# NVIDIA/tacotron2

Hardware: NVIDIA H100
Metric: mel frames/sec (B=64,T_text=150) (higher is better)
Workload: dtype f32 (split-fp16 tensor-core operands hi+lo, fp32 accumulate and state)

## Files before the change

tacotron2_b200/_engine.py:

```python
import contextlib
import ctypes as C
import threading

import torch

from . import _capi


def weight_table_spec(hp):
    E, K = hp.encoder_embedding_dim, hp.encoder_kernel_size
    s = [("embedding.weight", (hp.n_symbols, hp.symbols_embedding_dim))]

    def bn(p, c):
        return [(p + "weight", (c,)), (p + "bias", (c,)), (p + "running_mean", (c,)),
                (p + "running_var", (c,)), (p + "num_batches_tracked", ())]
    for i in range(hp.encoder_n_convolutions):
        p = "encoder.convolutions.%d." % i
        s += [(p + "0.conv.weight", (E, E, K)), (p + "0.conv.bias", (E,))] + bn(p + "1.", E)
    H = E // 2
    for suf in ("", "_reverse"):
        s += [("encoder.lstm.weight_ih_l0" + suf, (4 * H, E)), ("encoder.lstm.weight_hh_l0" + suf, (4 * H, H)),
              ("encoder.lstm.bias_ih_l0" + suf, (4 * H,)), ("encoder.lstm.bias_hh_l0" + suf, (4 * H,))]
    d = "decoder."
    nm = hp.n_mel_channels * hp.n_frames_per_step
# ... 278 lines not shown
        a.seed = next_seed() if seed is None else seed
        if stash is not None:
            a.stash, a.stash_bytes = stash.data_ptr(), stash.numel()
        a.gate_threshold = float(gate_threshold)
        a.score_mask_value = float(score_mask_value)
        a.mel, a.gate, a.align = mel.data_ptr(), gate.data_ptr(), align.data_ptr()
        a.mel_lengths, a.n_steps = mel_lengths.data_ptr(), n_steps.data_ptr()
        a.ws, a.ws_bytes = ws.data_ptr(), ws.numel()
        with torch.cuda.device(self.device):
            _capi.check(L.t2_decoder_run(self.handle, C.byref(a), self._stream()))
        self._last_decoder_args = (a, memory, len32, teacher_prenet, pk, ak, dk, ws, mel, gate, align, mel_lengths, n_steps)
        return mel, gate, align, mel_lengths, n_steps

    def decoder_stream(self, memory, n_steps_cap, prenet_keep=None, gate_threshold=0.5, score_mask_value=-float("inf"),
                       impl=None, seed=None):
        return DecoderStream(self, memory, n_steps_cap, prenet_keep, gate_threshold, score_mask_value,
                             self.impl if impl is None else impl, next_seed() if seed is None else seed)

    def decoder_profile(self):
        a = self._last_decoder_args[0]
        out = (C.c_int64 * 72)()
        _capi.check(_capi.lib().t2_decoder_profile(C.byref(a), out))
        names = ["E0 x2->att gemm", "E0 epilogue(ah)", "B1", "E1 ah->dec/att/q gemm", "B2", "attention", "B3",
                 "E2 ctx gemm", "E2 epilogue(dh)", "B4", "E3 dh gemm", "E3 epilogue(mel/x1)", "B5", "E4 x1 gemm+epi", "B6",
                 "att:im2col", "att:mma", "att:energies", "att:softmax", "att:context"]
        return {names[i]: [int(out[s * 24 + i]) for s in range(3)] for i in range(len(names))}

    def grad_table(self, named_grads):
        ptrs = (C.c_void_p * _capi.T2_NUM_WEIGHTS)()
        for i, (n, _) in enumerate(self.spec):
            t = named_grads.get(n)
            ptrs[i] = t.data_ptr() if t is not None else None
        return ptrs

    def decoder_stash(self, B, T_enc, T_mel):
        return self.stash_buffer("decoder", B, T_enc, T_mel)

    def decoder_backward(self, memory, memory_lengths, teacher_prenet, align, stash, seed, training, att_keep, dec_keep,
                         score_mask_value, d_mel, d_gate, d_align, named_grads):
        L = _capi.lib()
        B, Te = int(memory.shape[0]), int(memory.shape[1])
        T = int(align.shape[1])
        f32 = dict(device=self.device, dtype=torch.float32)
        d_memory = torch.empty(B, Te, self.hp.encoder_embedding_dim, **f32)
        d_prenet = torch.empty(T, B, self.hp.prenet_dim, **f32)
        ws = self._workspace("dec_bwd", L.t2_decoder_backward_workspace_bytes(self.handle, B, Te, T))
        a = _capi.T2DecoderBwdArgs()
        memory = memory.contiguous()
# ... 143 lines not shown
```

tacotron2_b200/csrc/decoder_persistent.cu:

```cuda
#include <stdlib.h>
#include <string.h>

#include <vector>

#include "decoder.h"
#include "gemm_f32.cuh"
#include "umma.cuh"

namespace t2 {

namespace {

constexpr int kG = 128;
constexpr int kThreads = 512;
constexpr int kStages = 4;
constexpr int kMaxStages = 4;
constexpr int kRows = 64;
constexpr int kXChunkBytes = 2 * kRows * kChunkK * 2;
constexpr int kColA = 0, kColD = 32, kColS = 64;
constexpr int kHiCols = 80;
constexpr int kAccPitch = 84;
constexpr int kAccBytes = kRows * kAccPitch * 4;
constexpr int kMmaWgs = 3;
constexpr int kAttRound = 64;
constexpr int kAttPlane = kAttRound * 128;
constexpr int kPaPitch = kAttRound + 4;
constexpr int kPaBytes = kAtt * kPaPitch * 4;
constexpr int kWStageMax = 2 * kHiCols * kChunkK * 2;
constexpr int kStageBytes = kXChunkBytes + kWStageMax;
constexpr int kNumEvents = 5;
constexpr int kPCols = 344;
constexpr int kQCta0 = 0, kQCtas = 16, kX2Cta0 = 16, kX2Ctas = 32, kPCta0 = 48, kPCtas = 43;
constexpr int kWeffBytes = kAtt * kChunkK * 2 * 2;
constexpr unsigned long long kWatchdogCycles = 1ull << 32;

struct EventPlan {
  uint32_t w_off;
  uint32_t w_bytes;
  int32_t nrows;
  int32_t col0;
  int32_t ncons;
  int32_t n[3];
  int32_t chunks;
};
struct CtaPlan {
  EventPlan ev[kNumEvents];
};

struct BwdCta {
  EventPlan ep;
  int32_t chunk0, nchunks;
  int32_t col0, split;
};

struct PersistentPack {
  uint8_t* wimg = nullptr; size_t wimg_bytes = 0;
  CtaPlan* plans = nullptr;
  float* wp_all = nullptr;
  float* bias_p = nullptr;
  float* bias_a = nullptr;
  float* bias_d = nullptr;
  int32_t* rows = nullptr;
  float* weff = nullptr;
  uint8_t* weff_img = nullptr;
  uint8_t* bwd_wimg[2] = {nullptr, nullptr};
  struct BwdCta* bwd_plans[2] = {nullptr, nullptr};
};

__global__ void fuse_prenet_proj_kernel(const float* __restrict__ w1, const float* __restrict__ wp,
                                        const float* __restrict__ bp, float* __restrict__ out_w,
                                        float* __restrict__ out_b) {
  const int r = blockIdx.x;
  for (int c = threadIdx.x; c < kDRnn + kEnc; c += blockDim.x) {
    float s = 0.f;
    for (int k = 0; k < kMel; ++k) s = fmaf(w1[r * kMel + k], wp[(long)k * (kDRnn + kEnc) + c], s);
    out_w[(long)r * (kDRnn + kEnc) + c] = s;
  }
  if (threadIdx.x == 0) {
    float s = 0.f;
    for (int k = 0; k < kMel; ++k) s = fmaf(w1[r * kMel + k], bp[k], s);
    out_b[r] = s;
  }
}

__global__ void fuse_location_kernel(const float* __restrict__ wld, const float* __restrict__ wloc,
// ... 78 lines not shown
  while (!ptx::mbar_try_wait(bar, parity)) {
    if (clock64() - t0 > kWatchdogCycles) watchdog_trap(ctrl, code);
  }
}

__device__ __forceinline__ void arrive_release(unsigned int* cnt) {
  asm volatile("fence.acq_rel.gpu;" ::: "memory");
  asm volatile("red.relaxed.gpu.global.add.u32 [%0], 1;" ::"l"(cnt) : "memory");
}
__device__ __forceinline__ void poll_acquire(unsigned int* cnt, unsigned int target, DecoderCtrl* ctrl, int code) {
  const unsigned long long t0 = clock64();
  while (true) {
    unsigned int c;
    asm volatile("ld.relaxed.gpu.global.u32 %0, [%1];" : "=r"(c) : "l"(cnt) : "memory");
    if ((int)(c - target) >= 0) break;
    if (clock64() - t0 > kWatchdogCycles) watchdog_trap(ctrl, code);
  }
  asm volatile("fence.acq_rel.gpu;" ::: "memory");
}

__device__ __forceinline__ void grid_barrier(DecoderCtrl* ctrl, unsigned int& target) {
  ptx::fence_proxy_async();
  __syncthreads();
  target += gridDim.x;
  if (threadIdx.x == 0) {
    arrive_release(&ctrl->bar_count);
    poll_acquire(&ctrl->bar_count, target, ctrl, 100);
  }
  __syncthreads();
  ptx::fence_proxy_async();
}

__device__ __forceinline__ void grid_arrive(DecoderCtrl* ctrl, unsigned int& target) {
  ptx::fence_proxy_async();
  __syncthreads();
  target += gridDim.x;
  if (threadIdx.x == 0) {
    arrive_release(&ctrl->bar_count);
  }
}
__device__ __forceinline__ void grid_wait(DecoderCtrl* ctrl, unsigned int target) {
  if (threadIdx.x == 0) {
    poll_acquire(&ctrl->bar_count, target, ctrl, 101);
  }
  __syncthreads();
  ptx::fence_proxy_async();
}

constexpr unsigned int kStopFlag = 1u << 24;
__device__ __forceinline__ void signal_counter(unsigned int* cnt, unsigned int inc) {
  ptx::fence_proxy_async();
  __syncthreads();
  if (threadIdx.x == 0) {
    asm volatile("fence.acq_rel.gpu;" ::: "memory");
    asm volatile("red.relaxed.gpu.global.add.u32 [%0], %1;" ::"l"(cnt), "r"(inc) : "memory");
  }
}
__device__ __forceinline__ bool wait_counter(unsigned int* cnt, unsigned int target, int* s_flag, DecoderCtrl* ctrl, int code) {
  if (threadIdx.x == 0) {
// ... 30 lines not shown
  uint8_t* stage0;
  __device__ __forceinline__ uint8_t* stage(uint32_t s) const { return stage0 + s * kStageBytes; }
  uint64_t* full;
  uint64_t* empty;
  uint32_t p_stage, p_phase;
  uint32_t c_stage, c_phase;
  uint64_t pol_x, pol_w;
  uint32_t pre;
  uint32_t ns;
};

__device__ __forceinline__ void prefetch_weights(Ring& rg, const EventPlan& nx, const uint8_t* w_img,
                                                 DecoderCtrl* ctrl) {
  uint32_t s = rg.p_stage, ph = rg.p_phase;
  const uint32_t n = min(rg.ns, (uint32_t)nx.chunks);
  for (uint32_t i = 0; i < n; ++i) {
    mbar_wait(&rg.empty[s], ph ^ 1, ctrl, 205);
    ptx::mbar_arrive_expect_tx(&rg.full[s], kXChunkBytes + nx.w_bytes);
    ptx::bulk_g2s_hint(rg.stage(s) + kXChunkBytes, w_img + nx.w_off + (size_t)i * nx.w_bytes, nx.w_bytes,
                       &rg.full[s], rg.pol_w);
    if (++s == rg.ns) { s = 0; ph ^= 1; }
  }
  rg.pre = n;
}

inline bool event_plan_fits(const EventPlan& ep, bool all_widths) {
  if (ep.ncons < 1 || ep.ncons > kMmaWgs) return false;
  for (int c = 0; c < ep.ncons; ++c)
    if (ep.n[c] != 16 && ep.n[c] != 32 && !(all_widths && (ep.n[c] == 8 || ep.n[c] == 24))) return false;
  return true;
}
inline void plan_one_matrix(EventPlan& ep, int rows) {
  ep.ncons = 0; ep.nrows = rows;
  for (int r = rows; r > 0 && ep.ncons < 3; ) {
    const int n = ep.ncons < 2 && r >= 32 ? 32 : r;
    ep.n[ep.ncons++] = n; r -= n;
  }
  ep.w_bytes = (uint32_t)rows * 256;
}
__device__ __forceinline__ void plan_image_rows(const EventPlan& ep, int r, int& hi, int& lo) {
  int roff = 0;
  for (int c = 0; c < ep.ncons; ++c) {
    if (r < ep.n[c]) { hi = roff + r; lo = hi + ep.n[c]; return; }
    r -= ep.n[c]; roff += 2 * ep.n[c];
  }
  hi = lo = 0;
// ... 113 lines not shown
}

__device__ __forceinline__ void acc_take8(float* s_acc, int row, int base, int col, float* s) {
  float* a = s_acc + row * kAccPitch + base + col;
#pragma unroll
  for (int i = 0; i < 8; ++i) { s[i] = a[i]; a[i] = 0.f; }
}

__device__ __forceinline__ void stash_lstm(float* gates, float* cs, float* hs, int t, int Btot, int b, int unit0,
                                           const float (&sg)[4][2], const float (&c)[2], const float (&h)[2]) {
  float* gp = gates + ((long)t * Btot + b) * (4 * kARnn) + unit0;
#pragma unroll
  for (int g = 0; g < 4; ++g) *reinterpret_cast<float2*>(gp + g * kARnn) = make_float2(sg[g][0], sg[g][1]);
  const long o = ((long)(t + 1) * Btot + b) * kARnn + unit0;
  *reinterpret_cast<float2*>(cs + o) = make_float2(c[0], c[1]);
  *reinterpret_cast<float2*>(hs + o) = make_float2(h[0], h[1]);
}

struct KParams {
  const CtaPlan* plans;
  const uint8_t* wimg;
  const float* bias_a; const float* bias_d; const float* bias_p;
  const uint8_t* weff_img; const float* w_v;
  const float* memory; const float* pm; const int32_t* mem_len;
  const uint8_t* prenet_keep; const uint8_t* att_keep; const uint8_t* dec_keep;
  uint8_t* x2_img; uint8_t* ah_img; uint8_t* ctx_img; uint8_t* dh_img; uint8_t* x1_img;
  const uint8_t* teacher_x2_img;
  float* q;
  float* mel; float* gate; float* align; int32_t* mel_lengths; int32_t* n_steps;
  DecoderCtrl* ctrl;
  int B, T, cap, infer, training;
  int nstages;
  int b0, Btot;
  float gate_threshold, score_mask_value, p_att, p_dec;
  uint64_t seed;
  DecoderStash st;
  int t_begin, t_end;
  float* rs_acc;
  float* rs_cell;
  float* rs_att;
  int32_t* rs_done;
  int32_t* rs_status;
};

__device__ __forceinline__ void store_split2(uint8_t* img, int row, int k, float v0, float v1) {
  const int chunk = k >> 6, kc = k & 63;
  __half h0, l0, h1, l1;
  split_fp16(v0, h0, l0);
  split_fp16(v1, h1, l1);
  __half* hi = reinterpret_cast<__half*>(img + (size_t)chunk * kXChunkBytes);
  __half* lo = hi + kRows * kChunkK;
  const uint32_t e = img_elem_offset(row, kc);
  *reinterpret_cast<__half2*>(hi + e) = __halves2half2(h0, h1);
  *reinterpret_cast<__half2*>(lo + e) = __halves2half2(l0, l1);
}

__global__ void __launch_bounds__(kThreads, 1) decoder_persistent_kernel(const KParams p) {
  extern __shared__ __align__(1024) uint8_t smem_raw[];
  const int tid = threadIdx.x, warp = tid >> 5, lane = tid & 31;
  const int cta = blockIdx.x;
  const int T = p.T, TP = T + kLocK - 1;
  const int ntiles = (T + 127) >> 7;

  uint8_t* sp = smem_raw;
  Ring rg;
  rg.ns = (uint32_t)p.nstages;
  rg.stage0 = sp; sp += p.nstages * kStageBytes;
  uint8_t* s_weff = sp; sp += kWeffBytes;
  float* s_acc = reinterpret_cast<float*>(sp); sp += kAccBytes;
  uint64_t* bars = reinterpret_cast<uint64_t*>(sp); sp += 16 * sizeof(uint64_t);
  rg.full = bars; rg.empty = bars + kMaxStages;
  int* s_live = reinterpret_cast<int*>(sp); sp += 16;
  int* s_flag = s_live + 1;
  float* s_bias_a = reinterpret_cast<float*>(sp); sp += 32 * 4;
  float* s_bias_d = reinterpret_cast<float*>(sp); sp += 32 * 4;
  float* s_v = reinterpret_cast<float*>(sp); sp += kAtt * 4;
  float* s_q = reinterpret_cast<float*>(sp); sp += kAtt * 4;
  float* s_red = reinterpret_cast<float*>(sp); sp += 32 * 4;
  uint32_t* s_mask = reinterpret_cast<uint32_t*>(sp); sp += kRows * 4;
  float* s_bias_p = reinterpret_cast<float*>(sp); sp += 8 * 4;
  long long* s_prof = reinterpret_cast<long long*>(sp); sp += 24 * 8;
  float* s_pad0 = reinterpret_cast<float*>(sp); sp += ((TP + 3) & ~3) * 4;
  float* s_pad1 = reinterpret_cast<float*>(sp); sp += ((TP + 3) & ~3) * 4;
// ... 23 lines not shown
    s_pad0[i] = resume ? p.rs_att[((size_t)cta * 2 + 0) * tpp + i] : 0.f;
    s_pad1[i] = resume ? p.rs_att[((size_t)cta * 2 + 1) * tpp + i] : 0.f;
  }
  const CtaPlan& plan = p.plans[cta];
  DecoderCtrl* ctrl = p.ctrl;
  const bool has_p = cta >= kPCta0 && cta < kPCta0 + kPCtas;
  const bool gate_cta = has_p && (cta - kPCta0) * 8 <= kMel && (cta - kPCta0) * 8 + 8 > kMel;
  if (resume && gate_cta && tid < p.B) ctrl->done[tid] = p.rs_done[tid];
  ptx::fence_proxy_async();
  __syncthreads();

  unsigned int bar_target = 0;
  const int quad = warp & 3, cg = warp >> 2;
  const int row = (quad & 1) * 32 + lane;
  const bool is_lo = quad >= 2;
  const bool erow = !is_lo && row < p.B;
  float c_att[2] = {0.f, 0.f}, c_dec[2] = {0.f, 0.f};
  float4* rs_cell = resume ? reinterpret_cast<float4*>(p.rs_cell) + ((size_t)cta * 4 + cg) * kRows + row : nullptr;
  if (resume && !is_lo) {
    const float4 c = *rs_cell;
    c_att[0] = c.x; c_att[1] = c.y; c_dec[0] = c.z; c_dec[1] = c.w;
  }
  const bool has_q = cta >= kQCta0 && cta < kQCta0 + kQCtas;
  const bool has_x2 = cta >= kX2Cta0 && cta < kX2Cta0 + kX2Ctas;
  const int halfk = (kLocK - 1) / 2;
  const int prof_slot = cta == 0 ? 0 : (cta == 60 ? 1 : (cta == 100 ? 2 : -1));
  long long prof_last = clock64();
  if (tid < 24) s_prof[tid] = 0;
#define T2_PROF(ph)                                                        \
  do {                                                                     \
    if (prof_slot >= 0 && tid == 0) {                                      \
      const long long now_ = clock64();                                    \
      s_prof[ph] += now_ - prof_last;    \
      prof_last = now_;                                                    \
    }                                                                      \
  } while (0)
#define T2_TAKE_GATES(colbase, g)                          \
  do {                                                     \
    if (!is_lo) acc_take8(s_acc, row, (colbase), cg * 8, g); \
  } while (0)

  auto x2_epilogue = [&]() {
    float g[8];
    if (cg == 0 && !is_lo) acc_take8(s_acc, row, kColS, 0, g);
    if (cg == 0 && erow) {
      const int col0 = (cta - kX2Cta0) * 8;
      float r[8];
      const uint32_t bits = s_mask[row];
#pragma unroll
      for (int j = 0; j < 8; ++j)
        r[j] = ((bits >> j) & 1u) ? fmaxf(g[j], 0.f) * 2.f : 0.f;
#pragma unroll
      for (int j = 0; j < 8; j += 2) store_split2(p.x2_img, row, col0 + j, r[j], r[j + 1]);
    }
  };

  int t = p.t_begin;
  for (; t < p.t_end; ++t) {
    {
      const uint8_t* x2 = p.infer ? p.x2_img : p.teacher_x2_img + (size_t)t * 4 * kXChunkBytes;
      run_event(rg, plan.ev[0], x2, p.wimg, 4, s_acc, ctrl, &plan.ev[1]);
      T2_PROF(0);
      float g[8];
      T2_TAKE_GATES(kColA, g);
      if (erow) {
        float hv[2], sg[4][2];
#pragma unroll
        for (int u = 0; u < 2; ++u) {
          const float* b = s_bias_a + (cg * 2 + u) * 4;
          const float gi = sigmoid_fast(g[u * 4 + 0] + b[0]);
          const float gf = sigmoid_fast(g[u * 4 + 1] + b[1]);
          const float gg = tanh_fast(g[u * 4 + 2] + b[2]);
          const float go = sigmoid_fast(g[u * 4 + 3] + b[3]);
          c_att[u] = gf * c_att[u] + gi * gg;
          float h = go * tanh_fast(c_att[u]);
          if (p.training) {
            const int unit = cta * 8 + cg * 2 + u;
            const long idx = (long)(p.b0 + row) * kARnn + unit;
            const bool keep = p.att_keep ? p.att_keep[(long)t * p.Btot * kARnn + idx] != 0
                                         : philox_keep(p.seed, t * 4 + 2, idx, p.p_att);
            h = keep ? h * (1.f / (1.f - p.p_att)) : 0.f;
          }
          hv[u] = h;
          sg[0][u] = gi; sg[1][u] = gf; sg[2][u] = gg; sg[3][u] = go;
        }
        store_split2(p.ah_img, row, cta * 8 + cg * 2, hv[0], hv[1]);
        if (p.st.ga) stash_lstm(p.st.ga, p.st.ca, p.st.ha, t, p.Btot, p.b0 + row, cta * 8 + cg * 2, sg, c_att, hv);
      }
      T2_PROF(1);
      signal_counter(&ctrl->ah_count[cta >> 3], 1u);
      T2_PROF(2);
    }
    {
      if (p.infer && is_lo && cg == 0 && row < p.B && t + 1 < p.cap && (has_p || has_x2)) {
        uint32_t bits = 0;
        if (has_x2) {
          const int col0 = (cta - kX2Cta0) * 8;
          if (p.prenet_keep) {
            const uint8_t* kp = p.prenet_keep + ((long)(t + 1) * 2 + 1) * p.Btot * kPre + (long)(p.b0 + row) * kPre + col0;
            for (int j = 0; j < 8; ++j) bits |= (kp[j] != 0 ? 1u : 0u) << j;
          } else {
            bits = philox_keep8(p.seed, (t + 1) * 4 + 1, (uint64_t)(p.b0 + row) * kPre + col0, 0.5f);
          }
        } else {
          const int pc0 = (cta - kPCta0) * 8;
          for (int j = 0; j < 8; ++j) {
            const int col = pc0 + j - (kMel + 1);
            if (col < 0 || col >= kPre) continue;
            const long idx = (long)(p.b0 + row) * kPre + col;
            const bool keep = p.prenet_keep ? p.prenet_keep[((long)(t + 1) * 2 + 0) * p.Btot * kPre + idx] != 0
                                            : philox_keep(p.seed, (t + 1) * 4 + 0, idx, 0.5f);
            bits |= (keep ? 1u : 0u) << j;
          }
        }
        s_mask[row] = bits;
      }
      run_event(rg, plan.ev[1], p.ah_img, p.wimg, 16, s_acc, ctrl, nullptr,
                ctrl->ah_count, 8u * (unsigned int)(t + 1 - p.t_begin));
      if (has_q && cg == 0 && !is_lo) {
        float g[8];
        acc_take8(s_acc, row, kColS, 0, g);
        if (erow) {
#pragma unroll
          for (int j = 0; j < 8; ++j) p.q[row * kAtt + (cta - kQCta0) * 8 + j] = g[j];
        }
      }
      T2_PROF(3);
    }
    const bool att_cta = (cta & 63) < p.B;
    const int att_b = cta & 63, ahalf = cta >> 6;
    uint8_t* aimg = rg.stage0;
    const int att_rounds = (T + kAttRound - 1) / kAttRound;
    const int img_bytes = 2 * kAttPlane;
    float* s_pa = reinterpret_cast<float*>(aimg + img_bytes);
    const int smem_rows = min(T, (p.nstages * kStageBytes - img_bytes - kPaBytes) / (kEnc / 2 * 4));
    auto att_im2col_mma_tr = [&](int r0) {
// ... 168 lines not shown
          acc.x = fmaf(a, m.x, acc.x); acc.y = fmaf(a, m.y, acc.y); acc.z = fmaf(a, m.z, acc.z); acc.w = fmaf(a, m.w, acc.w);
        }
        __syncthreads();
        float* scr = reinterpret_cast<float*>(rg.stage0);
        *reinterpret_cast<float4*>(scr + jg * (kEnc / 2) + c4 * 4) = acc;
        __syncthreads();
        if (tid < kEnc / 4) {
          const int col = tid * 2;
          float v0 = 0.f, v1 = 0.f;
#pragma unroll
          for (int g = 0; g < 8; ++g) { v0 += scr[g * (kEnc / 2) + col]; v1 += scr[g * (kEnc / 2) + col + 1]; }
          store_split2(p.ctx_img, b, ahalf * (kEnc / 2) + col, v0, v1);
          if (p.st.ga)
            *reinterpret_cast<float2*>(p.st.ctx + ((long)(t + 1) * p.Btot + p.b0 + b) * kEnc + ahalf * (kEnc / 2) + col) =
                make_float2(v0, v1);
        }
      }
      T2_PROF(19);
    }
    T2_PROF(5);
    grid_barrier(ctrl, bar_target);
    T2_PROF(6);
    {
      run_event(rg, plan.ev[2], p.ctx_img, p.wimg, 8, s_acc, ctrl, &plan.ev[3]);
      T2_PROF(7);
      float g[8];
      T2_TAKE_GATES(kColD, g);
      if (erow) {
        float hv[2], sg[4][2];
#pragma unroll
        for (int u = 0; u < 2; ++u) {
          const float* b = s_bias_d + (cg * 2 + u) * 4;
          const float gi = sigmoid_fast(g[u * 4 + 0] + b[0]);
          const float gf = sigmoid_fast(g[u * 4 + 1] + b[1]);
          const float gg = tanh_fast(g[u * 4 + 2] + b[2]);
          const float go = sigmoid_fast(g[u * 4 + 3] + b[3]);
          c_dec[u] = gf * c_dec[u] + gi * gg;
          float h = go * tanh_fast(c_dec[u]);
          if (p.training) {
            const int unit = cta * 8 + cg * 2 + u;
            const long idx = (long)(p.b0 + row) * kDRnn + unit;
            const bool keep = p.dec_keep ? p.dec_keep[(long)t * p.Btot * kDRnn + idx] != 0
                                         : philox_keep(p.seed, t * 4 + 3, idx, p.p_dec);
            h = keep ? h * (1.f / (1.f - p.p_dec)) : 0.f;
          }
          hv[u] = h;
          sg[0][u] = gi; sg[1][u] = gf; sg[2][u] = gg; sg[3][u] = go;
        }
        store_split2(p.dh_img, row, cta * 8 + cg * 2, hv[0], hv[1]);
        if (p.st.ga) stash_lstm(p.st.gd, p.st.cd, p.st.hd, t, p.Btot, p.b0 + row, cta * 8 + cg * 2, sg, c_dec, hv);
      }
      T2_PROF(8);
      signal_counter(&ctrl->dh_count[cta >> 3], 1u);
      T2_PROF(9);
    }
    {
      run_event(rg, plan.ev[3], p.dh_img, p.wimg, 16, s_acc, ctrl,
                (!p.infer && t + 1 < p.cap) ? &plan.ev[0] : nullptr,
                ctrl->dh_count, 8u * (unsigned int)(t + 1 - p.t_begin));
      T2_PROF(10);
      if (tid == 0) *s_live = 0;
      float g[8];
      if (has_p && cg == 0 && !is_lo) acc_take8(s_acc, row, kColS, 0, g);
      __syncthreads();
      if (has_p && cg == 0 && erow) {
        const int pc0 = (cta - kPCta0) * 8;
#pragma unroll
        for (int j = 0; j < 8; ++j) {
          const int pc = pc0 + j;
          const float v = g[j] + s_bias_p[j];
          if (pc < kMel) {
            p.mel[((long)row * p.cap + t) * kMel + pc] = v;
          } else if (pc == kMel) {
            p.gate[(long)row * p.cap + t] = v;
            if (p.infer) {
              int done = ctrl->done[row];
              if (!done && sigmoid_exact(v) > p.gate_threshold) {
                done = 1; ctrl->done[row] = 1; p.mel_lengths[row] = t + 1;
              }
              if (!done) atomicAdd(s_live, 1);
            }
          } else if (pc < kMel + 1 + kPre) {
            const int col = pc - (kMel + 1);
            float r = fmaxf(v, 0.f);
            if (p.infer && t + 1 < p.cap) r = ((s_mask[row] >> j) & 1u) ? r * 2.f : 0.f;
            if (p.infer) {
              __half h, l;
              split_fp16(r, h, l);
              __half* hi = reinterpret_cast<__half*>(p.x1_img + (size_t)(col >> 6) * kXChunkBytes);
              __half* lo = hi + kRows * kChunkK;
              const uint32_t e = img_elem_offset(row, col & 63);
              hi[e] = h; lo[e] = l;
            }
          }
        }
      }
      __syncthreads();
      if (gate_cta && tid == 0) atomicMax(p.n_steps, t + 1);
      T2_PROF(11);
      if (!p.infer) continue;
      bool stop = t + 1 == p.cap;
      if (has_p) signal_counter(&ctrl->x1_count, 1u + ((gate_cta && *s_live == 0) ? kStopFlag : 0u));
      if (has_x2) {
        stop |= wait_counter(&ctrl->x1_count, (unsigned int)(kPCtas * (t + 1 - p.t_begin)), s_flag, ctrl, 102);
        if (!stop) {
          run_event(rg, plan.ev[4], p.x1_img, p.wimg, 4, s_acc, ctrl, nullptr);
          x2_epilogue();
        }
        signal_counter(&ctrl->x2_count, 1u + (stop ? kStopFlag : 0u));
      }
      T2_PROF(12);
      stop |= wait_counter(&ctrl->x2_count, (unsigned int)(kX2Ctas * (t + 1 - p.t_begin)), s_flag, ctrl, 103);
      T2_PROF(14);
      if (stop) { ++t; break; }
    }
  }
  if (prof_slot >= 0 && tid == 0)
    for (int i = 0; i < 24; ++i) ctrl->prof[prof_slot][i] = s_prof[i];
  if (resume) {
    for (int i = tid; i < kRows * kAccPitch; i += kThreads) p.rs_acc[(size_t)cta * kRows * kAccPitch + i] = s_acc[i];
    for (int i = tid; i < TP; i += kThreads) {
      p.rs_att[((size_t)cta * 2 + 0) * tpp + i] = s_pad0[i];
      p.rs_att[((size_t)cta * 2 + 1) * tpp + i] = s_pad1[i];
    }
    if (!is_lo) *rs_cell = make_float4(c_att[0], c_att[1], c_dec[0], c_dec[1]);
    if (gate_cta && tid < p.B) p.rs_done[tid] = ctrl->done[tid];
  }
  if (cta == 0) {
    __syncthreads();
    const int ns = p.infer ? t : p.cap;
    bool ended = true;
    if (resume) ended = t >= p.cap || __syncthreads_count(tid < p.B && !__ldcg(&ctrl->done[tid])) == 0;
    if (ended) {
      for (int b = tid; b < p.B; b += kThreads)
        if (!p.infer || !__ldcg(&ctrl->done[b])) p.mel_lengths[b] = ns;
      if (tid == 0) atomicMax(p.n_steps, ns);
    }
    if (resume && tid == 0) { p.rs_status[0] = t; p.rs_status[1] = ended ? 1 : 0; }
  }
}

// ... 3 lines not shown
  const int TP = T + kLocK - 1;
  const int ntiles = (T + 127) / 128;
  const size_t att = (size_t)5 * ntiles * 128 * 4;
  return (size_t)nstages * kStageBytes + kWeffBytes + kAccBytes + 16 * 8 + 16 + 2 * 32 * 4 + kAtt * 4 + kAtt * 4 + 32 * 4 +
         kRows * 4 + 32 + 24 * 8 + 2 * (size_t)((TP + 3) & ~3) * 4 + att + 1024;
}
constexpr size_t kSmemLimit = 227 * 1024;
static int persistent_stages(int T) {
  int want = 4;
  const char* e = getenv("T2_STAGES");
  if (e && atoi(e) >= 3 && atoi(e) <= kMaxStages) want = atoi(e);
  while (want > 3 && persistent_smem_bytes(T, want) > kSmemLimit) --want;
  return want;
}

size_t persistent_ws_bytes(int B, int T, int cap) {
  (void)B; (void)T;
  return (size_t)(4 + 16 + 8 + 16 + 4) * kXChunkBytes + (size_t)kRows * kAtt * 4 + 1024 +
         (size_t)cap * 4 * kXChunkBytes;
}

bool persistent_supported(const T2Model* m, const T2DecoderArgs* a) {
  if (!m->pk) return false;
  if (m->sm_count < kG) return false;
  if (persistent_smem_bytes(a->T_enc, 3) > kSmemLimit) return false;
  return true;
}

int persistent_pack_create(T2Model* m, cudaStream_t s) {
  PersistentPack* pk = (PersistentPack*)m->pk;
  if (!pk) { pk = new PersistentPack(); m->pk = pk; }
  const int kdc = kDRnn + kEnc;
  std::vector<CtaPlan> plans(kG);
  size_t off = 0;
  for (int c = 0; c < kG; ++c) {
    const bool hq = c >= kQCta0 && c < kQCta0 + kQCtas, hx = c >= kX2Cta0 && c < kX2Cta0 + kX2Ctas,
               hp = c >= kPCta0 && c < kPCta0 + kPCtas;
    CtaPlan& pl = plans[c];
    memset(&pl, 0, sizeof(pl));
    auto set = [&](int ev, int chunks, int col0, std::initializer_list<int> ns) {
      EventPlan& e = pl.ev[ev];
      e.ncons = 0; e.nrows = 0; e.col0 = col0;
      for (int n : ns) { e.n[e.ncons++] = n; e.nrows += n; }
      e.w_bytes = (uint32_t)e.nrows * 256;
      e.w_off = (uint32_t)off;
      e.chunks = chunks;
      off += (size_t)chunks * e.w_bytes;
    };
    set(0, 4, kColA, {32});
    if (hq) set(1, 16, kColA, {32, 32, 16}); else set(1, 16, kColA, {32, 32});
    if (hp) set(2, 8, kColA, {32, 32, 16}); else set(2, 8, kColA, {32, 32});
    if (hp) set(3, 16, kColD, {32, 16}); else set(3, 16, kColD, {32});
    if (hx) set(4, 4, kColS, {16}); else { pl.ev[4].w_off = (uint32_t)off; }
    for (int ev = 0; ev < kNumEvents; ++ev)
      if (pl.ev[ev].nrows != 0 && !event_plan_fits(pl.ev[ev], false)) return fail(T2_ERR_INVALID, "event plan does not fit the MMA warpgroups");
  }
  if (off >= (size_t)4 << 30) return fail(T2_ERR_INVALID, "W image too large");
  if (!pk->wimg) {
    pk->wimg_bytes = off + 1024;
    T2_CUDA(cudaMalloc((void**)&pk->wimg, pk->wimg_bytes));
    T2_CUDA(cudaMalloc((void**)&pk->plans, sizeof(CtaPlan) * kG));
    T2_CUDA(cudaMalloc((void**)&pk->wp_all, (size_t)kPCols * kdc * 4));
    T2_CUDA(cudaMalloc((void**)&pk->bias_p, (size_t)kPCols * 4));
    T2_CUDA(cudaMalloc((void**)&pk->bias_a, (size_t)kG * 32 * 4));
    T2_CUDA(cudaMalloc((void**)&pk->bias_d, (size_t)kG * 32 * 4));
    T2_CUDA(cudaMalloc((void**)&pk->rows, (size_t)4 * kG * 32 * 4));
    T2_CUDA(cudaMalloc((void**)&pk->weff, (size_t)kAtt * kChunkK * 4));
    T2_CUDA(cudaMalloc((void**)&pk->weff_img, (size_t)kWeffBytes));
  }
  fuse_location_kernel<<<kAtt, kChunkK, 0, s>>>(m->w[W_ATT_LOC_DENSE], m->w[W_ATT_LOC_CONV], pk->weff);
  T2_LAUNCH_CHECK();
  pack_rows_image_kernel<<<1, 256, 0, s>>>(pk->weff, kAtt, kChunkK, pk->weff_img);
  T2_LAUNCH_CHECK();
  T2_CUDA(cudaMemcpyAsync(pk->plans, plans.data(), sizeof(CtaPlan) * kG, cudaMemcpyHostToDevice, s));
  T2_CUDA(cudaStreamSynchronize(s));
  T2_CUDA(cudaMemsetAsync(pk->wp_all, 0, (size_t)kPCols * kdc * 4, s));
  T2_CUDA(cudaMemsetAsync(pk->bias_p, 0, (size_t)kPCols * 4, s));
  T2_CUDA(cudaMemcpyAsync(pk->wp_all, m->projgate_w, (size_t)(kMel + 1) * kdc * 4, cudaMemcpyDeviceToDevice, s));
  T2_CUDA(cudaMemcpyAsync(pk->bias_p, m->projgate_b, (size_t)(kMel + 1) * 4, cudaMemcpyDeviceToDevice, s));
  fuse_prenet_proj_kernel<<<kPre, 256, 0, s>>>(m->w[W_PRENET0], m->w[W_PROJ_W], m->w[W_PROJ_B],
                                               pk->wp_all + (size_t)(kMel + 1) * kdc, pk->bias_p + kMel + 1);
  T2_LAUNCH_CHECK();
  pack_lstm_bias_kernel<<<(kG * 32 + 255) / 256, 256, 0, s>>>(m->arnn_b, pk->bias_a);
  T2_LAUNCH_CHECK();
  pack_lstm_bias_kernel<<<(kG * 32 + 255) / 256, 256, 0, s>>>(m->drnn_b, pk->bias_d);
  T2_LAUNCH_CHECK();
  std::vector<int32_t> rows((size_t)4 * kG * 32, -1);
  for (int c = 0; c < kG; ++c) {
    for (int col = 0; col < 32; ++col) rows[(0 * kG + c) * 32 + col] = (col & 3) * 1024 + c * 8 + (col >> 2);
    if (c >= kQCta0 && c < kQCta0 + kQCtas) for (int j = 0; j < 8; ++j) rows[(1 * kG + c) * 32 + j] = (c - kQCta0) * 8 + j;
    if (c >= kPCta0 && c < kPCta0 + kPCtas) for (int j = 0; j < 8; ++j) rows[(2 * kG + c) * 32 + j] = (c - kPCta0) * 8 + j;
    if (c >= kX2Cta0 && c < kX2Cta0 + kX2Ctas) for (int j = 0; j < 8; ++j) rows[(3 * kG + c) * 32 + j] = (c - kX2Cta0) * 8 + j;
  }
  T2_CUDA(cudaMemcpyAsync(pk->rows, rows.data(), rows.size() * 4, cudaMemcpyHostToDevice, s));
  T2_CUDA(cudaStreamSynchronize(s));
  const int32_t* r_lstm = pk->rows; const int32_t* r_q = pk->rows + kG * 32;
  const int32_t* r_p = pk->rows + 2 * kG * 32; const int32_t* r_x2 = pk->rows + 3 * kG * 32;
  auto pack = [&](const float* src, int ld, int kcol0, int chunks, const int32_t* rt, int ev, int cons) -> int {
    pack_consumer_kernel<<<dim3(chunks, kG), 256, 0, s>>>(src, ld, kcol0, rt, pk->plans, ev, cons, pk->wimg);
    T2_LAUNCH_CHECK();
    return T2_OK;
  };
  T2_TRY(pack(m->w[W_ARNN_WIH], kPre + kEnc, 0, 4, r_lstm, 0, 0));
  T2_TRY(pack(m->w[W_ARNN_WHH], kARnn, 0, 16, r_lstm, 1, 0));
  T2_TRY(pack(m->w[W_DRNN_WIH], kdc, 0, 16, r_lstm, 1, 1));
  T2_TRY(pack(m->w[W_ATT_QUERY], kARnn, 0, 16, r_q, 1, 2));
  T2_TRY(pack(m->w[W_ARNN_WIH], kPre + kEnc, kPre, 8, r_lstm, 2, 0));
  T2_TRY(pack(m->w[W_DRNN_WIH], kdc, kARnn, 8, r_lstm, 2, 1));
  T2_TRY(pack(pk->wp_all, kdc, kDRnn, 8, r_p, 2, 2));
  T2_TRY(pack(m->w[W_DRNN_WHH], kDRnn, 0, 16, r_lstm, 3, 0));
  T2_TRY(pack(pk->wp_all, kdc, 0, 16, r_p, 3, 1));
  T2_TRY(pack(m->w[W_PRENET1], kPre, 0, 4, r_x2, 4, 0));
  return T2_OK;
}

void persistent_pack_destroy(T2Model* m) {
  PersistentPack* pk = (PersistentPack*)m->pk;
  if (!pk) return;
  cudaFree(pk->wimg); cudaFree(pk->plans); cudaFree(pk->wp_all); cudaFree(pk->bias_p);
  cudaFree(pk->bias_a); cudaFree(pk->bias_d); cudaFree(pk->rows); cudaFree(pk->weff); cudaFree(pk->weff_img);
  for (int i = 0; i < 2; ++i) { cudaFree(pk->bwd_wimg[i]); cudaFree(pk->bwd_plans[i]); }
  delete pk;
  m->pk = nullptr;
}

static int run_persistent_slice(T2Model* m, const T2DecoderArgs* a, cudaStream_t s, int b0, int nb);

int decoder_run_persistent(T2Model* m, const T2DecoderArgs* a, cudaStream_t s) {
  T2_CUDA(cudaMemsetAsync(a->n_steps, 0, sizeof(int32_t), s));
  for (int b0 = 0; b0 < a->B; b0 += kRows) {
    const int nb = a->B - b0 < kRows ? a->B - b0 : kRows;
    T2_TRY(run_persistent_slice(m, a, s, b0, nb));
  }
  return T2_OK;
}

constexpr size_t kImagesBytes = (size_t)(4 + 16 + 8 + 16 + 4) * kXChunkBytes + (size_t)kRows * kAtt * 4;

static int processed_memory(T2Model* m, const T2DecoderArgs* a, int b0, int nb, float* pm, cudaStream_t s) {
  GemmArgs g;
  g.seg[0] = {a->memory + (size_t)b0 * a->T_enc * kEnc, kEnc, m->w[W_ATT_MEMORY], kEnc, kEnc};
  g.M = nb * a->T_enc; g.N = kAtt; g.C = pm; g.ldc = kAtt;
  return gemm_f32(g, s);
}

static void slice_params(T2Model* m, const T2DecoderArgs* a, int b0, int nb, KParams* pp) {
  PersistentPack* pk = (PersistentPack*)m->pk;
  KParams& p = *pp;
  const int T = a->T_enc, cap = a->n_steps_cap;
  memset(&p, 0, sizeof(p));
  p.plans = pk->plans; p.wimg = pk->wimg; p.bias_a = pk->bias_a; p.bias_d = pk->bias_d; p.bias_p = pk->bias_p;
  p.weff_img = pk->weff_img; p.w_v = m->w[W_ATT_V];
  p.memory = a->memory + (size_t)b0 * T * kEnc;
  p.mem_len = a->memory_lengths ? a->memory_lengths + b0 : nullptr;
  p.prenet_keep = a->prenet_keep; p.att_keep = a->att_keep; p.dec_keep = a->dec_keep;
  p.mel = a->mel + (size_t)b0 * cap * kMel; p.gate = a->gate + (size_t)b0 * cap; p.align = a->align + (size_t)b0 * cap * T;
  p.mel_lengths = a->mel_lengths + b0; p.n_steps = a->n_steps;
  p.b0 = b0; p.Btot = a->B;
  p.B = nb; p.T = T; p.cap = cap; p.infer = a->mode == T2_MODE_INFER; p.training = a->training;
  p.gate_threshold = a->gate_threshold; p.score_mask_value = a->score_mask_value;
  p.p_att = m->cfg.p_attention_dropout; p.p_dec = m->cfg.p_decoder_dropout; p.seed = a->seed;
  p.t_begin = 0; p.t_end = cap;
}

static void carve_images(uint8_t* img, KParams* p) {
  p->x2_img = img; img += 4 * kXChunkBytes;
  p->ah_img = img; img += 16 * kXChunkBytes;
  p->ctx_img = img; img += 8 * kXChunkBytes;
  p->dh_img = img; img += 16 * kXChunkBytes;
  p->x1_img = img; img += 4 * kXChunkBytes;
  p->q = (float*)img;
}

static int launch_persistent(KParams& p, cudaStream_t s) {
  p.nstages = persistent_stages(p.T);
  const size_t smem = persistent_smem_bytes(p.T, p.nstages);
  T2_CUDA(cudaFuncSetAttribute(decoder_persistent_kernel, cudaFuncAttributeMaxDynamicSharedMemorySize, (int)smem));
  cudaLaunchConfig_t cfg;
  memset(&cfg, 0, sizeof(cfg));
  cfg.gridDim = dim3(kG); cfg.blockDim = dim3(kThreads); cfg.dynamicSmemBytes = smem; cfg.stream = s;
  cudaLaunchAttribute attr;
  attr.id = cudaLaunchAttributeCooperative; attr.val.cooperative = 1;
  cfg.attrs = &attr; cfg.numAttrs = 1;
  const cudaError_t le = cudaLaunchKernelEx(&cfg, decoder_persistent_kernel, p);
  if (le != cudaSuccess) return fail(T2_ERR_CUDA, "persistent decoder launch failed: %s", cudaGetErrorString(le));
  if (getenv("T2_VERBOSE")) fprintf(stderr, "[t2b200] persistent decoder: B=%d T_enc=%d cap=%d stages=%d smem=%zu steps=%d-%d\n",
                                    p.B, p.T, p.cap, p.nstages, smem, p.t_begin, p.t_end);
  g_launch_count++;
  return T2_OK;
}

static int run_persistent_slice(T2Model* m, const T2DecoderArgs* a, cudaStream_t s, int b0, int nb) {
  const int T = a->T_enc, cap = a->n_steps_cap;
  DecoderWs w;
  T2_TRY(decoder_ws_carve(a, &w));
  T2_CUDA(cudaMemsetAsync(w.ctrl, 0, sizeof(DecoderCtrl), s));
  T2_CUDA(cudaMemsetAsync(w.persistent, 0, kImagesBytes, s));
  T2_TRY(processed_memory(m, a, b0, nb, w.pm, s));
  KParams p;
  slice_params(m, a, b0, nb, &p);
  carve_images((uint8_t*)w.persistent, &p);
  p.pm = w.pm;
  p.ctrl = w.ctrl;
// ... 281 lines not shown
```

Measured before the change: 799,400.

## Move prenet layer-2 GEMM to dedicated role CTAs and reorder DRNN W_hh event

Adds four extra CTAs to the persistent grid that only compute the second prenet layer (x1->x2) with their own smem-resident weight image. Previously 32 of the 128 main CTAs did this work in a serialized wait-compute-signal step. Those CTAs now run the decoder W_hh GEMM as a separate event after the x1 signal, so they overlap with the role CTAs. This needs 132 SMs (exactly H100's count). It also changes barrier accounting to exclude the role CTAs and adds a prefetch drain on stop.

```diff
diff --git a/tacotron2_b200/_engine.py b/tacotron2_b200/_engine.py
--- a/tacotron2_b200/_engine.py
+++ b/tacotron2_b200/_engine.py
@@ -324,8 +324,10 @@
         out = (C.c_int64 * 72)()
         _capi.check(_capi.lib().t2_decoder_profile(C.byref(a), out))
         names = ["E0 x2->att gemm", "E0 epilogue(ah)", "B1", "E1 ah->dec/att/q gemm", "B2", "attention", "B3",
-                 "E2 ctx gemm", "E2 epilogue(dh)", "B4", "E3 dh gemm", "E3 epilogue(mel/x1)", "B5", "E4 x1 gemm+epi", "B6",
-                 "att:im2col", "att:mma", "att:energies", "att:softmax", "att:context"]
+                 "E2 ctx gemm", "E2 epilogue(dh)", "B4", "E3 dh gemm", "E3 epilogue(mel/x1)", "x1 signal",
+                 "E3r dh->W_hh gemm (split plan)", "x2 wait",
+                 "att:im2col", "att:mma", "att:energies", "att:softmax", "att:context",
+                 "role:x2 keep bits", "role:x1 wait", "role:E4 x1->x2", "role:x2 signal"]
         return {names[i]: [int(out[s * 24 + i]) for s in range(3)] for i in range(len(names))}
 
     def grad_table(self, named_grads):
diff --git a/tacotron2_b200/csrc/decoder_persistent.cu b/tacotron2_b200/csrc/decoder_persistent.cu
--- a/tacotron2_b200/csrc/decoder_persistent.cu
+++ b/tacotron2_b200/csrc/decoder_persistent.cu
@@ -12,6 +12,12 @@
 namespace {
 
 constexpr int kG = 128;
+constexpr int kRoleCtas = 4;
+constexpr int kGrid = kG + kRoleCtas;
+constexpr int kRoleCols = kPre / kRoleCtas;
+static_assert(kRoleCols == kChunkK, "a role CTA owns exactly one x2 image chunk");
+constexpr int kRoleWChunk = 32 * 256;
+constexpr int kRoleWBytes = 2 * 4 * kRoleWChunk;
 constexpr int kThreads = 512;
 constexpr int kStages = 4;
 constexpr int kMaxStages = 4;
@@ -30,7 +36,7 @@
 constexpr int kStageBytes = kXChunkBytes + kWStageMax;
 constexpr int kNumEvents = 5;
 constexpr int kPCols = 344;
-constexpr int kQCta0 = 0, kQCtas = 16, kX2Cta0 = 16, kX2Ctas = 32, kPCta0 = 48, kPCtas = 43;
+constexpr int kQCta0 = 0, kQCtas = 16, kPCta0 = 48, kPCtas = 43;
 constexpr int kWeffBytes = kAtt * kChunkK * 2 * 2;
 constexpr unsigned long long kWatchdogCycles = 1ull << 32;
 
@@ -61,6 +67,7 @@
   float* bias_a = nullptr;
   float* bias_d = nullptr;
   int32_t* rows = nullptr;
+  uint8_t* w2_img = nullptr;
   float* weff = nullptr;
   uint8_t* weff_img = nullptr;
   uint8_t* bwd_wimg[2] = {nullptr, nullptr};
@@ -185,7 +192,7 @@
 __device__ __forceinline__ void grid_barrier(DecoderCtrl* ctrl, unsigned int& target) {
   ptx::fence_proxy_async();
   __syncthreads();
-  target += gridDim.x;
+  target += kG;
   if (threadIdx.x == 0) {
     arrive_release(&ctrl->bar_count);
     poll_acquire(&ctrl->bar_count, target, ctrl, 100);
@@ -197,7 +204,7 @@
 __device__ __forceinline__ void grid_arrive(DecoderCtrl* ctrl, unsigned int& target) {
   ptx::fence_proxy_async();
   __syncthreads();
-  target += gridDim.x;
+  target += kG;
   if (threadIdx.x == 0) {
     arrive_release(&ctrl->bar_count);
   }
@@ -274,6 +281,19 @@
     if (++s == rg.ns) { s = 0; ph ^= 1; }
   }
   rg.pre = n;
+}
+
+__device__ __forceinline__ void drain_prefetch(Ring& rg, const uint8_t* x_img, DecoderCtrl* ctrl) {
+  if (threadIdx.x == 0) {
+    uint32_t s = rg.p_stage, ph = rg.p_phase;
+    for (uint32_t i = 0; i < rg.pre; ++i) {
+      ptx::bulk_g2s_hint(rg.stage(s), x_img + (size_t)i * kXChunkBytes, kXChunkBytes, &rg.full[s], rg.pol_x);
+      mbar_wait(&rg.full[s], ph, ctrl, 208);
+      if (++s == rg.ns) { s = 0; ph ^= 1; }
+    }
+    rg.pre = 0;
+  }
+  __syncthreads();
 }
 
 inline bool event_plan_fits(const EventPlan& ep, bool all_widths) {
@@ -433,6 +453,7 @@
   const uint8_t* wimg;
   const float* bias_a; const float* bias_d; const float* bias_p;
   const uint8_t* weff_img; const float* w_v;
+  const uint8_t* w2_img;
   const float* memory; const float* pm; const int32_t* mem_len;
   const uint8_t* prenet_keep; const uint8_t* att_keep; const uint8_t* dec_keep;
   uint8_t* x2_img; uint8_t* ah_img; uint8_t* ctx_img; uint8_t* dh_img; uint8_t* x1_img;
@@ -466,10 +487,108 @@
   *reinterpret_cast<__half2*>(lo + e) = __halves2half2(l0, l1);
 }
 
+__device__ __forceinline__ void prenet2_role_cta(const KParams& p, uint8_t* smem) {
+  const int tid = threadIdx.x, warp = tid >> 5;
+  const int r = blockIdx.x - kG, col0 = r * kRoleCols;
+  DecoderCtrl* ctrl = p.ctrl;
+  uint8_t* s_w2 = smem;
+  uint8_t* s_x1 = s_w2 + kRoleWBytes;
+  uint64_t* s_full = reinterpret_cast<uint64_t*>(s_x1 + 4 * kXChunkBytes);
+  uint8_t* s_keep = reinterpret_cast<uint8_t*>(s_full + 4);
+  int* s_flag = reinterpret_cast<int*>(s_keep + kRows * 8);
+  for (int i = tid; i < kRoleWBytes / 16; i += kThreads)
+    reinterpret_cast<uint4*>(s_w2)[i] = reinterpret_cast<const uint4*>(p.w2_img + (size_t)r * kRoleWBytes)[i];
+  if (tid == 0) {
+    for (int i = 0; i < 4; ++i) ptx::mbar_init(&s_full[i], 1);
+    ptx::fence_barrier_init();
+  }
+  const uint64_t pol_x = ptx::policy_evict_last();
+  ptx::fence_proxy_async();
+  __syncthreads();
+  uint32_t phase = 0;
+  const bool prof = r == 0 && tid == 0;
+  long long prof_acc[4] = {0, 0, 0, 0}, prof_last = clock64();
+  auto prof_mark = [&](int i) {
+    if (prof) { const long long now = clock64(); prof_acc[i] += now - prof_last; prof_last = now; }
+  };
+  for (int t = p.t_begin; t < p.t_end; ++t) {
+    if (t + 1 < p.cap) {
+      const int row = tid >> 3, c = col0 + (tid & 7) * 8;
+      uint32_t bits = 0;
+      if (row < p.B) {
+        if (p.prenet_keep) {
+          const uint8_t* kp = p.prenet_keep + ((long)(t + 1) * 2 + 1) * p.Btot * kPre + (long)(p.b0 + row) * kPre + c;
+          for (int j = 0; j < 8; ++j) bits |= (kp[j] != 0 ? 1u : 0u) << j;
+        } else {
+          bits = philox_keep8(p.seed, (t + 1) * 4 + 1, (uint64_t)(p.b0 + row) * kPre + c, 0.5f);
+        }
+      }
+      s_keep[tid] = (uint8_t)bits;
+    }
+    prof_mark(0);
+    bool stop = t + 1 == p.cap;
+    stop |= wait_counter(&ctrl->x1_count, (unsigned int)(kPCtas * (t + 1 - p.t_begin)), s_flag, ctrl, 102);
+    prof_mark(1);
+    if (!stop) {
+      if (tid == 0)
+        for (int i = 0; i < 4; ++i) {
+          ptx::mbar_arrive_expect_tx(&s_full[i], kXChunkBytes);
+          ptx::bulk_g2s_hint(s_x1 + i * kXChunkBytes, p.x1_img + (size_t)i * kXChunkBytes, kXChunkBytes, &s_full[i], pol_x);
+        }
+      if (warp >= 4 && warp < 12) {
+        const int cons = (warp >> 2) - 1, wt = tid & 127;
+        float d[32];
+#pragma unroll
+        for (int i = 0; i < 32; ++i) d[i] = 0.f;
+#pragma unroll 1
+        for (int i = 0; i < 4; ++i) {
+          mbar_wait(&s_full[i], phase, ctrl, 207);
+          const uint32_t xs = ptx::smem_u32(s_x1 + i * kXChunkBytes);
+          const uint32_t ws = ptx::smem_u32(s_w2 + (cons * 4 + i) * kRoleWChunk);
+          ptx::wg_fence_regs<32>(d);
+          ptx::wg_fence();
+#pragma unroll
+          for (int kk = 0; kk < kChunkK / 16; ++kk) {
+            const uint64_t b = ptx::make_sw128_desc(ws + kk * 32);
+            ptx::wgmma_f16<64>(d, ptx::make_sw128_desc(xs + kk * 32), b);
+            ptx::wgmma_f16<64>(d, ptx::make_sw128_desc(xs + kRows * 128 + kk * 32), b);
+          }
+          ptx::wg_commit();
+          ptx::wg_wait<0>();
+          ptx::wg_fence_regs<32>(d);
+        }
+#pragma unroll
+        for (int j = 0; j < 16; j += 2) {
+          const int row = ptx::wg_frag_row(j, wt), c = cons * 32 + ptx::wg_frag_col(j, wt);
+          float g0 = 0.f, g1 = 0.f;
+          g0 += d[j] + d[16 + j];
+          g1 += d[j + 1] + d[16 + j + 1];
+          const uint32_t bits = s_keep[row * 8 + (c >> 3)] >> (c & 7);
+          const float r0 = (bits & 1u) ? fmaxf(g0, 0.f) * 2.f : 0.f;
+          const float r1 = (bits & 2u) ? fmaxf(g1, 0.f) * 2.f : 0.f;
+          if (row < p.B) store_split2(p.x2_img, row, col0 + c, r0, r1);
+        }
+      }
+      phase ^= 1;
+    }
+    __syncthreads();
+    prof_mark(2);
+    signal_counter(&ctrl->x2_count, 1u + (stop ? kStopFlag : 0u));
+    prof_mark(3);
+    if (stop) break;
+  }
+  if (prof)
+    for (int i = 0; i < 4; ++i) ctrl->prof[2][20 + i] = prof_acc[i];
+}
+
 __global__ void __launch_bounds__(kThreads, 1) decoder_persistent_kernel(const KParams p) {
   extern __shared__ __align__(1024) uint8_t smem_raw[];
   const int tid = threadIdx.x, warp = tid >> 5, lane = tid & 31;
   const int cta = blockIdx.x;
+  if (cta >= kG) {
+    if (p.infer) prenet2_role_cta(p, smem_raw);
+    return;
+  }
   const int T = p.T, TP = T + kLocK - 1;
   const int ntiles = (T + 127) >> 7;
 
@@ -539,7 +658,6 @@
     c_att[0] = c.x; c_att[1] = c.y; c_dec[0] = c.z; c_dec[1] = c.w;
   }
   const bool has_q = cta >= kQCta0 && cta < kQCta0 + kQCtas;
-  const bool has_x2 = cta >= kX2Cta0 && cta < kX2Cta0 + kX2Ctas;
   const int halfk = (kLocK - 1) / 2;
   const int prof_slot = cta == 0 ? 0 : (cta == 60 ? 1 : (cta == 100 ? 2 : -1));
   long long prof_last = clock64();
@@ -556,21 +674,6 @@
   do {                                                     \
     if (!is_lo) acc_take8(s_acc, row, (colbase), cg * 8, g); \
   } while (0)
-
-  auto x2_epilogue = [&]() {
-    float g[8];
-    if (cg == 0 && !is_lo) acc_take8(s_acc, row, kColS, 0, g);
-    if (cg == 0 && erow) {
-      const int col0 = (cta - kX2Cta0) * 8;
-      float r[8];
-      const uint32_t bits = s_mask[row];
-#pragma unroll
-      for (int j = 0; j < 8; ++j)
-        r[j] = ((bits >> j) & 1u) ? fmaxf(g[j], 0.f) * 2.f : 0.f;
-#pragma unroll
-      for (int j = 0; j < 8; j += 2) store_split2(p.x2_img, row, col0 + j, r[j], r[j + 1]);
-    }
-  };
 
   int t = p.t_begin;
   for (; t < p.t_end; ++t) {
@@ -609,26 +712,16 @@
       T2_PROF(2);
     }
     {
-      if (p.infer && is_lo && cg == 0 && row < p.B && t + 1 < p.cap && (has_p || has_x2)) {
+      if (p.infer && is_lo && cg == 0 && row < p.B && t + 1 < p.cap && has_p) {
         uint32_t bits = 0;
-        if (has_x2) {
-          const int col0 = (cta - kX2Cta0) * 8;
-          if (p.prenet_keep) {
-            const uint8_t* kp = p.prenet_keep + ((long)(t + 1) * 2 + 1) * p.Btot * kPre + (long)(p.b0 + row) * kPre + col0;
-            for (int j = 0; j < 8; ++j) bits |= (kp[j] != 0 ? 1u : 0u) << j;
-          } else {
-            bits = philox_keep8(p.seed, (t + 1) * 4 + 1, (uint64_t)(p.b0 + row) * kPre + col0, 0.5f);
-          }
-        } else {
-          const int pc0 = (cta - kPCta0) * 8;
-          for (int j = 0; j < 8; ++j) {
-            const int col = pc0 + j - (kMel + 1);
-            if (col < 0 || col >= kPre) continue;
-            const long idx = (long)(p.b0 + row) * kPre + col;
-            const bool keep = p.prenet_keep ? p.prenet_keep[((long)(t + 1) * 2 + 0) * p.Btot * kPre + idx] != 0
-                                            : philox_keep(p.seed, (t + 1) * 4 + 0, idx, 0.5f);
-            bits |= (keep ? 1u : 0u) << j;
-          }
+        const int pc0 = (cta - kPCta0) * 8;
+        for (int j = 0; j < 8; ++j) {
+          const int col = pc0 + j - (kMel + 1);
+          if (col < 0 || col >= kPre) continue;
+          const long idx = (long)(p.b0 + row) * kPre + col;
+          const bool keep = p.prenet_keep ? p.prenet_keep[((long)(t + 1) * 2 + 0) * p.Btot * kPre + idx] != 0
+                                          : philox_keep(p.seed, (t + 1) * 4 + 0, idx, 0.5f);
+          bits |= (keep ? 1u : 0u) << j;
         }
         s_mask[row] = bits;
       }
@@ -843,7 +936,7 @@
     grid_barrier(ctrl, bar_target);
     T2_PROF(6);
     {
-      run_event(rg, plan.ev[2], p.ctx_img, p.wimg, 8, s_acc, ctrl, &plan.ev[3]);
+      run_event(rg, plan.ev[2], p.ctx_img, p.wimg, 8, s_acc, ctrl, has_p ? &plan.ev[3] : &plan.ev[4]);
       T2_PROF(7);
       float g[8];
       T2_TAKE_GATES(kColD, g);
@@ -875,10 +968,15 @@
       signal_counter(&ctrl->dh_count[cta >> 3], 1u);
       T2_PROF(9);
     }
+    const EventPlan* e0_next = t + 1 < p.t_end ? &plan.ev[0] : nullptr;
     {
-      run_event(rg, plan.ev[3], p.dh_img, p.wimg, 16, s_acc, ctrl,
-                (!p.infer && t + 1 < p.cap) ? &plan.ev[0] : nullptr,
-                ctrl->dh_count, 8u * (unsigned int)(t + 1 - p.t_begin));
+      if (has_p) {
+        run_event(rg, plan.ev[3], p.dh_img, p.wimg, 16, s_acc, ctrl, plan.ev[4].nrows ? &plan.ev[4] : e0_next,
+                  ctrl->dh_count, 8u * (unsigned int)(t + 1 - p.t_begin));
+      } else {
+        run_event(rg, plan.ev[4], p.dh_img, p.wimg, 16, s_acc, ctrl, e0_next, ctrl->dh_count,
+                  8u * (unsigned int)(t + 1 - p.t_begin));
+      }
       T2_PROF(10);
       if (tid == 0) *s_live = 0;
       float g[8];
@@ -919,25 +1017,23 @@
       __syncthreads();
       if (gate_cta && tid == 0) atomicMax(p.n_steps, t + 1);
       T2_PROF(11);
-      if (!p.infer) continue;
-      bool stop = t + 1 == p.cap;
+    }
+    bool stop = false;
+    if (p.infer) {
+      stop = t + 1 == p.cap;
       if (has_p) signal_counter(&ctrl->x1_count, 1u + ((gate_cta && *s_live == 0) ? kStopFlag : 0u));
-      if (has_x2) {
-        stop |= wait_counter(&ctrl->x1_count, (unsigned int)(kPCtas * (t + 1 - p.t_begin)), s_flag, ctrl, 102);
-        if (!stop) {
-          run_event(rg, plan.ev[4], p.x1_img, p.wimg, 4, s_acc, ctrl, nullptr);
-          x2_epilogue();
-        }
-        signal_counter(&ctrl->x2_count, 1u + (stop ? kStopFlag : 0u));
-      }
       T2_PROF(12);
-      stop |= wait_counter(&ctrl->x2_count, (unsigned int)(kX2Ctas * (t + 1 - p.t_begin)), s_flag, ctrl, 103);
+    }
+    if (has_p && plan.ev[4].nrows) run_event(rg, plan.ev[4], p.dh_img, p.wimg, 16, s_acc, ctrl, e0_next);
+    T2_PROF(13);
+    if (p.infer) {
+      stop |= wait_counter(&ctrl->x2_count, (unsigned int)(kRoleCtas * (t + 1 - p.t_begin)), s_flag, ctrl, 103);
       T2_PROF(14);
-      if (stop) { ++t; break; }
+      if (stop) { drain_prefetch(rg, p.x2_img, ctrl); ++t; break; }
     }
   }
   if (prof_slot >= 0 && tid == 0)
-    for (int i = 0; i < 24; ++i) ctrl->prof[prof_slot][i] = s_prof[i];
+    for (int i = 0; i < 20; ++i) ctrl->prof[prof_slot][i] = s_prof[i];
   if (resume) {
     for (int i = tid; i < kRows * kAccPitch; i += kThreads) p.rs_acc[(size_t)cta * kRows * kAccPitch + i] = s_acc[i];
     for (int i = tid; i < TP; i += kThreads) {
@@ -987,7 +1083,7 @@
 
 bool persistent_supported(const T2Model* m, const T2DecoderArgs* a) {
   if (!m->pk) return false;
-  if (m->sm_count < kG) return false;
+  if (m->sm_count < kGrid) return false;
   if (persistent_smem_bytes(a->T_enc, 3) > kSmemLimit) return false;
   return true;
 }
@@ -999,8 +1095,7 @@
   std::vector<CtaPlan> plans(kG);
   size_t off = 0;
   for (int c = 0; c < kG; ++c) {
-    const bool hq = c >= kQCta0 && c < kQCta0 + kQCtas, hx = c >= kX2Cta0 && c < kX2Cta0 + kX2Ctas,
-               hp = c >= kPCta0 && c < kPCta0 + kPCtas;
+    const bool hq = c >= kQCta0 && c < kQCta0 + kQCtas, hp = c >= kPCta0 && c < kPCta0 + kPCtas;
     CtaPlan& pl = plans[c];
     memset(&pl, 0, sizeof(pl));
     auto set = [&](int ev, int chunks, int col0, std::initializer_list<int> ns) {
@@ -1015,8 +1110,8 @@
     set(0, 4, kColA, {32});
     if (hq) set(1, 16, kColA, {32, 32, 16}); else set(1, 16, kColA, {32, 32});
     if (hp) set(2, 8, kColA, {32, 32, 16}); else set(2, 8, kColA, {32, 32});
-    if (hp) set(3, 16, kColD, {32, 16}); else set(3, 16, kColD, {32});
-    if (hx) set(4, 4, kColS, {16}); else { pl.ev[4].w_off = (uint32_t)off; }
+    if (hp) set(3, 16, kColS, {16}); else { pl.ev[3].w_off = (uint32_t)off; }
+    set(4, 16, kColD, {32});
     for (int ev = 0; ev < kNumEvents; ++ev)
       if (pl.ev[ev].nrows != 0 && !event_plan_fits(pl.ev[ev], false)) return fail(T2_ERR_INVALID, "event plan does not fit the MMA warpgroups");
   }
@@ -1029,7 +1124,8 @@
     T2_CUDA(cudaMalloc((void**)&pk->bias_p, (size_t)kPCols * 4));
     T2_CUDA(cudaMalloc((void**)&pk->bias_a, (size_t)kG * 32 * 4));
     T2_CUDA(cudaMalloc((void**)&pk->bias_d, (size_t)kG * 32 * 4));
-    T2_CUDA(cudaMalloc((void**)&pk->rows, (size_t)4 * kG * 32 * 4));
+    T2_CUDA(cudaMalloc((void**)&pk->rows, (size_t)3 * kG * 32 * 4));
+    T2_CUDA(cudaMalloc((void**)&pk->w2_img, (size_t)kRoleCtas * kRoleWBytes));
     T2_CUDA(cudaMalloc((void**)&pk->weff, (size_t)kAtt * kChunkK * 4));
     T2_CUDA(cudaMalloc((void**)&pk->weff_img, (size_t)kWeffBytes));
   }
@@ -1050,17 +1146,16 @@
   T2_LAUNCH_CHECK();
   pack_lstm_bias_kernel<<<(kG * 32 + 255) / 256, 256, 0, s>>>(m->drnn_b, pk->bias_d);
   T2_LAUNCH_CHECK();
-  std::vector<int32_t> rows((size_t)4 * kG * 32, -1);
+  std::vector<int32_t> rows((size_t)3 * kG * 32, -1);
   for (int c = 0; c < kG; ++c) {
     for (int col = 0; col < 32; ++col) rows[(0 * kG + c) * 32 + col] = (col & 3) * 1024 + c * 8 + (col >> 2);
     if (c >= kQCta0 && c < kQCta0 + kQCtas) for (int j = 0; j < 8; ++j) rows[(1 * kG + c) * 32 + j] = (c - kQCta0) * 8 + j;
     if (c >= kPCta0 && c < kPCta0 + kPCtas) for (int j = 0; j < 8; ++j) rows[(2 * kG + c) * 32 + j] = (c - kPCta0) * 8 + j;
-    if (c >= kX2Cta0 && c < kX2Cta0 + kX2Ctas) for (int j = 0; j < 8; ++j) rows[(3 * kG + c) * 32 + j] = (c - kX2Cta0) * 8 + j;
   }
   T2_CUDA(cudaMemcpyAsync(pk->rows, rows.data(), rows.size() * 4, cudaMemcpyHostToDevice, s));
   T2_CUDA(cudaStreamSynchronize(s));
   const int32_t* r_lstm = pk->rows; const int32_t* r_q = pk->rows + kG * 32;
-  const int32_t* r_p = pk->rows + 2 * kG * 32; const int32_t* r_x2 = pk->rows + 3 * kG * 32;
+  const int32_t* r_p = pk->rows + 2 * kG * 32;
   auto pack = [&](const float* src, int ld, int kcol0, int chunks, const int32_t* rt, int ev, int cons) -> int {
     pack_consumer_kernel<<<dim3(chunks, kG), 256, 0, s>>>(src, ld, kcol0, rt, pk->plans, ev, cons, pk->wimg);
     T2_LAUNCH_CHECK();
@@ -1073,9 +1168,13 @@
   T2_TRY(pack(m->w[W_ARNN_WIH], kPre + kEnc, kPre, 8, r_lstm, 2, 0));
   T2_TRY(pack(m->w[W_DRNN_WIH], kdc, kARnn, 8, r_lstm, 2, 1));
   T2_TRY(pack(pk->wp_all, kdc, kDRnn, 8, r_p, 2, 2));
-  T2_TRY(pack(m->w[W_DRNN_WHH], kDRnn, 0, 16, r_lstm, 3, 0));
-  T2_TRY(pack(pk->wp_all, kdc, 0, 16, r_p, 3, 1));
-  T2_TRY(pack(m->w[W_PRENET1], kPre, 0, 4, r_x2, 4, 0));
+  T2_TRY(pack(pk->wp_all, kdc, 0, 16, r_p, 3, 0));
+  T2_TRY(pack(m->w[W_DRNN_WHH], kDRnn, 0, 16, r_lstm, 4, 0));
+  for (int rc = 0; rc < 2 * kRoleCtas; ++rc) {
+    pack_rows_image_kernel<<<kPre / kChunkK, 256, 0, s>>>(m->w[W_PRENET1] + (size_t)rc * 32 * kPre, 32, kPre,
+                                                          pk->w2_img + (size_t)rc * 4 * kRoleWChunk);
+    T2_LAUNCH_CHECK();
+  }
   return T2_OK;
 }
 
@@ -1083,7 +1182,8 @@
   PersistentPack* pk = (PersistentPack*)m->pk;
   if (!pk) return;
   cudaFree(pk->wimg); cudaFree(pk->plans); cudaFree(pk->wp_all); cudaFree(pk->bias_p);
-  cudaFree(pk->bias_a); cudaFree(pk->bias_d); cudaFree(pk->rows); cudaFree(pk->weff); cudaFree(pk->weff_img);
+  cudaFree(pk->bias_a); cudaFree(pk->bias_d); cudaFree(pk->rows); cudaFree(pk->w2_img); cudaFree(pk->weff);
+  cudaFree(pk->weff_img);
   for (int i = 0; i < 2; ++i) { cudaFree(pk->bwd_wimg[i]); cudaFree(pk->bwd_plans[i]); }
   delete pk;
   m->pk = nullptr;
@@ -1115,7 +1215,7 @@
   const int T = a->T_enc, cap = a->n_steps_cap;
   memset(&p, 0, sizeof(p));
   p.plans = pk->plans; p.wimg = pk->wimg; p.bias_a = pk->bias_a; p.bias_d = pk->bias_d; p.bias_p = pk->bias_p;
-  p.weff_img = pk->weff_img; p.w_v = m->w[W_ATT_V];
+  p.weff_img = pk->weff_img; p.w_v = m->w[W_ATT_V]; p.w2_img = pk->w2_img;
   p.memory = a->memory + (size_t)b0 * T * kEnc;
   p.mem_len = a->memory_lengths ? a->memory_lengths + b0 : nullptr;
   p.prenet_keep = a->prenet_keep; p.att_keep = a->att_keep; p.dec_keep = a->dec_keep;
@@ -1143,7 +1243,7 @@
   T2_CUDA(cudaFuncSetAttribute(decoder_persistent_kernel, cudaFuncAttributeMaxDynamicSharedMemorySize, (int)smem));
   cudaLaunchConfig_t cfg;
   memset(&cfg, 0, sizeof(cfg));
-  cfg.gridDim = dim3(kG); cfg.blockDim = dim3(kThreads); cfg.dynamicSmemBytes = smem; cfg.stream = s;
+  cfg.gridDim = dim3(kGrid); cfg.blockDim = dim3(kThreads); cfg.dynamicSmemBytes = smem; cfg.stream = s;
   cudaLaunchAttribute attr;
   attr.id = cudaLaunchAttributeCooperative; attr.val.cooperative = 1;
   cfg.attrs = &attr; cfg.numAttrs = 1;
```

New measurement: 811,800, median of 6. 1.02x the previous value.
